# jaekor91/understanding-HMC

Hardware: AMD Instinct MI355X
Metric: leapfrog steps/sec (whole node) + ESS/sec, D=100 MVN at 1M chains (higher is better)
Workload: dtype f64

## Files before the change

understanding-hmc_amd/csrc/hmc_capi.cpp:

```cpp
#include <algorithm>
#include <cmath>
#include <cstdarg>
#include <cstdio>
#include <cstdlib>
#include <mutex>
#include <string>
#include <unordered_map>

#include "hmc.h"
#include "hmc_internal.hpp"
#include "hmc_logit.hpp"
#include "hmc_mix.hpp"

namespace {

thread_local std::string g_err;
#ifdef HMC_DEBUG_HOOKS
unsigned long long* g_stamps = nullptr;
int64_t g_stamp_waves = 0;
#endif

hmc_status fail(hmc_status st, const char* fmt, ...) {
  char buf[512];
  va_list ap;
// ... 163 lines not shown

}

extern "C" {

#ifdef HMC_DEBUG_HOOKS
int64_t hmc_debug_stamps(unsigned long long* host, int64_t cap_words) {
  if (!g_stamps) return 0;
  const int64_t words = g_stamp_waves * hmc::kStampWords < cap_words ? g_stamp_waves * hmc::kStampWords : cap_words;
  if (hipDeviceSynchronize() != hipSuccess) return 0;
  if (hipMemcpy(host, g_stamps, words * sizeof(unsigned long long), hipMemcpyDeviceToHost) != hipSuccess) return 0;
  return words;
}
#endif

const char* hmc_version(void) { return "hmc_amd 0.1.0 gfx950 (diag random kernels, C ABI v1)"; }

const char* hmc_last_error(void) { return g_err.c_str(); }

hmc_status hmc_chain_init(const hmc_target* t, const hmc_kinetic* k, const hmc_schedule* s, const hmc_replay* r,
                          const double* q_start, hmc_state* st, void* stream) {
  if (hmc_status e = check_schedule(t, k, s, false)) return e;
  if (!st) return fail(HMC_EINVAL, "null state");
  if (hmc_status e = check_mass(t, k, s)) return e;
  if (s->n_chains == 0) return HMC_OK;
  if (!st->q || !st->E_prev || !q_start) return fail(HMC_EINVAL, "null state/q_start");
  const bool replay = s->rng_mode == HMC_RNG_REPLAY;
  if (replay && (!r || !r->p0)) return fail(HMC_EINVAL, "replay mode needs p0");
  if (hmc_status e = ws_check(st->order, order_need(t, k, s, st), "hmc_chain_init: state.order")) return e;
  const bool dense = t->kind == HMC_TARGET_DENSE;
  if (hmc::big_path(dense, t->D)) {
    if (!st->order) return fail(HMC_EINVAL, "D=%d needs hmc_random_workspace_size() bytes in state.order", t->D);
    const hmc::Layout lay{0, 0, 0, (t->D + 1) / 2};
    hmc::RandArgs a = rand_args(t, k, s, replay ? r : nullptr, st, lay);
    a.qstart = q_start;
    return hip_status(hmc::launch_big_init(hmc::big_args(a, st->order, dense), dense, replay, (hipStream_t)stream),
                      "hmc_chain_init(large D)");
  }
  if (t->kind == HMC_TARGET_DENSE) {
    const hmc::Layout lay{0, 0, 0, (t->D + 1) / 2};
    hmc::RandArgs a = rand_args(t, k, s, replay ? r : nullptr, st, lay);
    a.qstart = q_start;
    if (st->order) {
      int32_t* valid = reinterpret_cast<int32_t*>(reinterpret_cast<char*>(st->order) +
                                                  hmc::dense_gcache_offset_bytes(s->n_chains) - 16);
      if (hmc_status e = hip_status(hipMemsetAsync(valid, 0, sizeof(int32_t), (hipStream_t)stream), "hmc_chain_init"))
        return e;
    }
    return hip_status(hmc::launch_dense_init(a, replay, (hipStream_t)stream), "hmc_chain_init(dense)");
  }
  const int L_lo = s->L_high > s->L_low ? s->L_low : 5, L_hi = s->L_high > s->L_low ? s->L_high : 20;
  const hmc::Layout lay = hmc::choose_layout(t->D, L_lo, L_hi);
  if (lay.K == 0) return fail(HMC_ENOTSUP, "D=%d too large for the diagonal kernels", t->D);
  hmc::RandArgs a = rand_args(t, k, s, replay ? r : nullptr, st, lay);
  a.qstart = q_start;
  return hip_status(hmc::launch_random_init(a, lay, general_diag(t, k), replay, (hipStream_t)stream),
                    "hmc_chain_init");
}

hmc_status hmc_random_iters(const hmc_target* t, const hmc_kinetic* k, const hmc_schedule* s, const hmc_replay* r,
                            hmc_state* st, void* stream) {
  if (hmc_status e = check_schedule(t, k, s, true)) return e;
  if (!st) return fail(HMC_EINVAL, "null state");
  if (hmc_status e = check_window(t, s, st)) return e;
  if (hmc_status e = check_mass(t, k, s)) return e;
  if (s->iter_begin < 1 || s->iter_end < s->iter_begin || s->iter_end > s->n_iter + 1)
    return fail(HMC_EINVAL, "iteration range must satisfy 1 <= begin <= end <= Niter+1");
  if (s->n_chains == 0) return HMC_OK;
  if (!st->q || !st->E_prev) return fail(HMC_EINVAL, "null state");
  const bool replay = s->rng_mode == HMC_RNG_REPLAY;
  if (replay && (!r || !r->p || !r->L || !r->lnu)) return fail(HMC_EINVAL, "replay mode needs p, L, lnu");
  if (s->n_chains == 0 || s->iter_end == s->iter_begin) return HMC_OK;
  if (st->n_save > 0 && st->traj_q && st->traj_stride < s->L_high)
    return fail(HMC_EINVAL, "traj_stride must be >= L_high");
  if (hmc_status e = ws_check(st->order, order_need(t, k, s, st), "hmc_random_iters: state.order")) return e;
  const bool dense = t->kind == HMC_TARGET_DENSE;
  if (hmc::big_path(dense, t->D)) {
    if (!st->order) return fail(HMC_EINVAL, "D=%d needs hmc_random_workspace_size() bytes in state.order", t->D);
    const hmc::Layout lay{0, 0, 0, (t->D + 1) / 2};
    hmc::RandArgs a = rand_args(t, k, s, replay ? r : nullptr, st, lay);
    return hip_status(hmc::launch_big_iters(hmc::big_args(a, st->order, dense), dense,
                                            s->fp_mode == HMC_MODE_EXACT, replay, (hipStream_t)stream),
                      "hmc_random_iters(large D)");
  }
  if (t->kind == HMC_TARGET_DENSE) {
    const hmc::Layout lay{0, 0, 0, (t->D + 1) / 2};
    hmc::RandArgs a = rand_args(t, k, s, replay ? r : nullptr, st, lay);
    const bool exact = s->fp_mode == HMC_MODE_EXACT;
    int32_t* gvalid = nullptr;
    if (st->order) {
      char* base = reinterpret_cast<char*>(st->order);
      gvalid = reinterpret_cast<int32_t*>(base + hmc::dense_gcache_offset_bytes(s->n_chains) - 16);
      a.gcache = reinterpret_cast<double*>(base + hmc::dense_gcache_offset_bytes(s->n_chains));
      a.gvalid = gvalid;
    }
    auto mark_valid = [&]() -> hmc_status {
      return gvalid ? hip_status(hipMemsetAsync(gvalid, 1, 1, (hipStream_t)stream), "hmc_random_iters") : HMC_OK;
    };
    if (!st->order || a.traj_q || !hmc::dense_order_ok(a)) {
      if (hmc_status e = hip_status(hmc::launch_dense_iters(a, exact, replay, (hipStream_t)stream),
                                    "hmc_random_iters(dense)"))
        return e;
      return mark_valid();
    }
    for (int it = s->iter_begin; it < s->iter_end; ++it) {
      if (hmc_status e = hip_status(hmc::launch_dense_order(a, it, replay, st->order, (hipStream_t)stream),
                                    "hmc_random_iters(dense order)"))
        return e;
      a.it0 = it;
      a.it1 = it + 1;
      a.order = st->order;
      if (hmc_status e = hip_status(hmc::launch_dense_iters(a, exact, replay, (hipStream_t)stream),
                                    "hmc_random_iters(dense)"))
        return e;
      if (hmc_status e = mark_valid()) return e;
    }
    return HMC_OK;
  }
  const hmc::Layout lay = hmc::choose_layout(t->D, s->L_low, s->L_high);
  if (lay.K == 0) return fail(HMC_ENOTSUP, "D=%d too large for the diagonal kernels", t->D);
  hmc::RandArgs a = rand_args(t, k, s, replay ? r : nullptr, st, lay);
  const int64_t lmax = std::max<int64_t>(std::max(s->L_high, 1), a.dbgL > 0 ? a.dbgL : 1);
  const int64_t chunk = std::max<int64_t>(1, 0x7FFFFFFFll / (lmax * lmax));
  for (int it = s->iter_begin; it < s->iter_end;) {
    const int end = (int)std::min<int64_t>(s->iter_end, it + chunk);
    a.it0 = it;
    a.it1 = end;
    if (hmc_status e = hip_status(hmc::launch_random_iters(a, lay, s->fp_mode == HMC_MODE_EXACT, general_diag(t, k),
                                                           replay, (hipStream_t)stream),
                                  "hmc_random_iters"))
      return e;
    it = end;
  }
  return HMC_OK;
}

int32_t hmc_random_leapfrog_form(const hmc_target* t, const hmc_kinetic* k, const hmc_schedule* s) {
  if (!t || !k || !s || t->D < 1 || t->kind == HMC_TARGET_DENSE || hmc::big_path(false, t->D)) return 0;
  const hmc::Layout lay = hmc::choose_layout(t->D, s->L_low, s->L_high);
  if (lay.K == 0) return 0;
  hmc::RandArgs a{};
  a.dt = k->dt;
  return hmc::leapfrog_three_term(a, lay, s->fp_mode == HMC_MODE_EXACT, general_diag(t, k)) ? 1 : 0;
}

hmc_status hmc_random_layout(const hmc_target* t, const hmc_schedule* s, int32_t out[4]) {
  if (!t || !s || !out) return fail(HMC_EINVAL, "hmc_random_layout: null target/schedule/out");
  if (t->D < 1) return fail(HMC_EINVAL, "D must be >= 1");
  if (s->L_high <= s->L_low) return fail(HMC_EINVAL, "L_low must be < L_high (randint)");
  if (t->kind == HMC_TARGET_DENSE) return fail(HMC_ENOTSUP, "hmc_random_layout: dense targets have no such layout");
  if (hmc::big_path(false, t->D)) return fail(HMC_ENOTSUP, "hmc_random_layout: D=%d runs the large-D path", t->D);
  const hmc::Layout lay = hmc::choose_layout(t->D, s->L_low, s->L_high);
  if (lay.K == 0) return fail(HMC_ENOTSUP, "D=%d too large for the diagonal kernels", t->D);
  out[0] = lay.K;
  out[1] = lay.lpc;
  out[2] = lay.cpw;
  out[3] = hmc::wave_layout(lay) ? 1 : 0;
  return HMC_OK;
}

int64_t hmc_random_workspace_size_ex(const hmc_target* t, const hmc_kinetic* k, int64_t n_chains) {
  if (!t || n_chains < 0 || t->D < 1) return 0;
  const bool dense = t->kind == HMC_TARGET_DENSE;
  if (hmc::big_path(dense, t->D)) return hmc::big_workspace_bytes(n_chains, t->D, dense, !k || k->minv_full);
  if (!dense) return 0;
  return hmc::dense_workspace_bytes(n_chains, t->D);
}

int64_t hmc_random_workspace_size(const hmc_target* t, int64_t n_chains) {
  return hmc_random_workspace_size_ex(t, nullptr, n_chains);
}

int64_t hmc_nuts_workspace_size_ex(int32_t D, int64_t n_chains, int32_t d_max, int32_t iters_per_call,
                                   int32_t philox_momenta) {
  if (D < 1 || n_chains < 0 || d_max < 1 || d_max > hmc::kNutsDmaxMax || iters_per_call < 1) return 0;
  int64_t doubles = 0;
  switch (hmc::nuts_kernel(D)) {
    case hmc::NutsKernel::Tree:
      doubles = hmc::nuts_ws_doubles(n_chains, D, d_max, philox_momenta ? iters_per_call : 0);
      break;
    case hmc::NutsKernel::Lock:
      doubles = hmc::nuts_lock_ws_doubles(n_chains, D, d_max, !philox_momenta);
      break;
    case hmc::NutsKernel::PerChain:
      doubles = hmc::nuts_big_ws_doubles(n_chains, D, d_max);
      break;
  }
  return doubles * (int64_t)sizeof(double);
}

int64_t hmc_nuts_workspace_size(int32_t D, int64_t n_chains, int32_t d_max) {
  return std::max(hmc_nuts_workspace_size_ex(D, n_chains, d_max, 32, 1),
                  hmc_nuts_workspace_size_ex(D, n_chains, d_max, 32, 0));
}

static int64_t nuts_need(const hmc_target* t, const hmc_kinetic* k, const hmc_schedule* s) {
  if (s->iter_end <= s->iter_begin || s->n_chains == 0) return 0;
  const int32_t pm = s->rng_mode == HMC_RNG_PHILOX && !k->minv_full ? 1 : 0;
  const int64_t need = hmc_nuts_workspace_size_ex(t->D, s->n_chains, s->d_max, s->iter_end - s->iter_begin, pm);
  return need > 0 ? need : -1;
}

hmc_status hmc_workspace_register(const void* workspace, int64_t bytes) {
  if (!workspace || bytes < 0) return fail(HMC_EINVAL, "hmc_workspace_register: null pointer or negative size");
  ws_record(workspace, bytes);
  return HMC_OK;
}

hmc_status hmc_chain_init_ws(const hmc_target* t, const hmc_kinetic* k, const hmc_schedule* s, const hmc_replay* r,
                             const double* q_start, hmc_state* st, int64_t order_bytes, void* stream) {
  if (hmc_status e = check_schedule(t, k, s, false)) return e;
  if (!st) return fail(HMC_EINVAL, "null state");
  if (!k) return fail(HMC_EINVAL, "null kinetic");
  const int64_t need = order_need(t, k, s, st);
  if (order_bytes < need)
    return fail(HMC_EINVAL, "hmc_chain_init_ws: state.order of %lld bytes, this call needs %lld "
                "(hmc_random_workspace_size_ex)", (long long)order_bytes, (long long)need);
  if (st->order) ws_record(st->order, order_bytes);
  return hmc_chain_init(t, k, s, r, q_start, st, stream);
}

hmc_status hmc_random_iters_ws(const hmc_target* t, const hmc_kinetic* k, const hmc_schedule* s, const hmc_replay* r,
                               hmc_state* st, int64_t order_bytes, void* stream) {
  if (hmc_status e = check_schedule(t, k, s, true)) return e;
  if (!st) return fail(HMC_EINVAL, "null state");
  if (!k) return fail(HMC_EINVAL, "null kinetic");
  const int64_t need = order_need(t, k, s, st);
  if (order_bytes < need)
    return fail(HMC_EINVAL, "hmc_random_iters_ws: state.order of %lld bytes, this call needs %lld "
                "(hmc_random_workspace_size_ex)", (long long)order_bytes, (long long)need);
  if (st->order) ws_record(st->order, order_bytes);
  return hmc_random_iters(t, k, s, r, st, stream);
}

hmc_status hmc_nuts_iters_ws(const hmc_target* t, const hmc_kinetic* k, const hmc_schedule* s, const hmc_replay* r,
                             hmc_state* st, void* workspace, int64_t workspace_bytes, void* stream) {
  if (hmc_status e = check_schedule(t, k, s, false)) return e;
  if (s->d_max < 1 || s->d_max > hmc::kNutsDmaxMax) return fail(HMC_EINVAL, "d_max must be in [1, %d]", hmc::kNutsDmaxMax);
  const int64_t need = nuts_need(t, k, s);
  if (need < 0) return fail(HMC_EINVAL, "NUTS workspace: unsupported D=%d / d_max=%d", t->D, s->d_max);
  if (workspace_bytes < need)
    return fail(HMC_EINVAL, "NUTS workspace of %lld bytes; this call (D=%d, %lld chains, d_max=%d, %d iterations, "
                "%s momenta) needs %lld (hmc_nuts_workspace_size_ex)", (long long)workspace_bytes, t->D,
                (long long)s->n_chains, s->d_max, s->iter_end - s->iter_begin,
                s->rng_mode == HMC_RNG_PHILOX && !k->minv_full ? "Philox" : "no pre-drawn", (long long)need);
  ws_record(workspace, workspace_bytes);
  return hmc_nuts_iters(t, k, s, r, st, workspace, stream);
}

hmc_status hmc_nuts_iters(const hmc_target* t, const hmc_kinetic* k, const hmc_schedule* s, const hmc_replay* r,
                          hmc_state* st, void* workspace, void* stream) {
  if (hmc_status e = check_schedule(t, k, s, false)) return e;
  if (!st) return fail(HMC_EINVAL, "null state");
  if (hmc_status e = check_window(t, s, st)) return e;
  if (s->iter_begin < 1 || s->iter_end < s->iter_begin || s->iter_end > s->n_iter + 1)
    return fail(HMC_EINVAL, "iteration range must satisfy 1 <= begin <= end <= Niter+1");
  if (s->n_chains == 0) return HMC_OK;
  if (!st->q || !st->E_prev) return fail(HMC_EINVAL, "null state");
  if (s->d_max < 1 || s->d_max > hmc::kNutsDmaxMax) return fail(HMC_EINVAL, "d_max must be in [1, %d]", hmc::kNutsDmaxMax);
  if (hmc_status e = check_mass(t, k, s)) return e;
  if (t->kind != HMC_TARGET_DENSE) return fail(HMC_ENOTSUP, "NUTS runs the dense kernel: pass prec as dense");
  const bool replay = s->rng_mode == HMC_RNG_REPLAY;
  if (replay && (!r || !r->p || !r->tape || r->tape_stride < 1)) return fail(HMC_EINVAL, "replay mode needs p and tape");
  if (s->n_chains == 0 || s->iter_end == s->iter_begin) return HMC_OK;
  if (!workspace) return fail(HMC_EINVAL, "null workspace");
  {
    const int64_t need = nuts_need(t, k, s);
    if (need < 0) return fail(HMC_EINVAL, "NUTS workspace: unsupported D=%d / d_max=%d", t->D, s->d_max);
    if (hmc_status e = ws_check(workspace, need, "hmc_nuts_iters: workspace")) return e;
  }
  const hmc::Layout lay{0, 0, 16, (t->D + 1) / 2};
  hmc::RandArgs a = rand_args(t, k, s, replay ? r : nullptr, st, lay);
  a.d_max = s->d_max;
  a.on_dmax = s->on_dmax;
  a.ws = static_cast<double*>(workspace);
  if (replay) {
    a.tape = r->tape;
    a.tape_stride = r->tape_stride;
  }
  a.traj_q = nullptr;
  a.n_save = 0;
  const bool exact = s->fp_mode == HMC_MODE_EXACT;
  switch (hmc::nuts_kernel(t->D)) {
    case hmc::NutsKernel::Lock:
      return hip_status(hmc::launch_nuts_lock(a, exact, replay, (hipStream_t)stream), "hmc_nuts_iters(lockstep)");
    case hmc::NutsKernel::PerChain:
      return hip_status(hmc::launch_nuts_big(a, exact, replay, (hipStream_t)stream), "hmc_nuts_iters(large D)");
    case hmc::NutsKernel::Tree:
      break;
  }
  return hip_status(hmc::launch_nuts_iters(a, exact, replay, (hipStream_t)stream), "hmc_nuts_iters");
}

hmc_status hmc_leapfrog(const hmc_target* t, const hmc_kinetic* k, int64_t n, const double* p, const double* q,
                        double* p_out, double* q_out, int32_t fp_mode, void* stream) {
  if (!t || !k || t->D < 1 || n < 0) return fail(HMC_EINVAL, "bad arguments");
  if (n > 0 && (!p || !q || !p_out || !q_out)) return fail(HMC_EINVAL, "null row pointers");
  if (p_out == p || q_out == q || p_out == q || q_out == p) return fail(HMC_EINVAL, "outputs alias inputs");
  hmc::RowArgs a{};
  a.n = n;
  a.D = t->D;
  a.dense = t->kind == HMC_TARGET_DENSE;
  a.q0 = t->q0;
  a.prec = t->prec;
  if (hmc_status e = check_mass(t, k, nullptr)) return e;
  a.minv = k->minv;
// ... 500 lines not shown
```

understanding-hmc_amd/csrc/hmc_internal.hpp:

```cpp
#pragma once
#include <hip/hip_runtime.h>
#include <stdint.h>

#include "hmc.h"

namespace hmc {

constexpr int kStampWords = 16;

struct Layout {
  int K;
  int lpc;
  int cpw;
  int npairs;
};

struct RandArgs {
  int64_t n;
  int64_t chain_offset;
  int D, npairs, lpc, cpw;
  int niter, wu, thin, Lc, L_low, L_high, it0, it1, i_oob;
  uint32_t k0, k1;
  double dt, h, logc;
  double lf_c, lf_ch, lf_idt2;
  const double* q0;
  const double* prec;
  const double* minv;
  const double* pscale;
  const double* dtv;
  const double* minvf;
  const double* cholt;
  const double* kick;
  const double* rp0;
  const double* rp;
  const double* rlnu;
  const int32_t* rL;
  const double* qstart;
  double* q;
  double* Eprev;
  double* qc;
  double* Ec;
  double* dEc;
  unsigned long long* cnt;
  double* traj_q;
  int32_t* traj_len;
  int32_t* decision;
  int n_save, traj_stride;
  int Lq, q_row0;
  int d_max, on_dmax;
  uint64_t wait_cap;
  int nuts_kb;
  double* ws;
  const double* tape;
  int64_t tape_stride;
  int dbg;
  int dbgL;
  unsigned long long* stamps;
  const int32_t* order;
  double* gcache;
  const int32_t* gvalid;
  int64_t ntiles;
};

using DenseArgs = RandArgs;
int dense_tiles(int D);
constexpr int kNutsDmaxMax = 30;
int64_t nuts_ws_doubles(int64_t n, int D, int d_max, int mom_iters);
hipError_t launch_nuts_iters(const RandArgs& a, bool exact, bool replay, hipStream_t s);
int64_t nuts_big_ws_doubles(int64_t n, int D, int d_max);
bool nuts_lock_path(int D);
int64_t nuts_lock_ws_doubles(int64_t n, int D, int d_max, bool mass);
hipError_t launch_nuts_lock(const RandArgs& a, bool exact, bool replay, hipStream_t s);
hipError_t launch_nuts_big(const RandArgs& a, bool exact, bool replay, hipStream_t s);
enum class NutsKernel { Tree, Lock, PerChain };
inline NutsKernel nuts_kernel(int D) {
  if (dense_tiles(D)) return NutsKernel::Tree;
  return nuts_lock_path(D) ? NutsKernel::Lock : NutsKernel::PerChain;
}

Layout choose_layout(int D, int L_low, int L_high);
bool wave_layout(const Layout& lay);

hipError_t launch_random_init(const RandArgs& a, const Layout& lay, bool gen, bool replay, hipStream_t s);
hipError_t launch_random_iters(const RandArgs& a, const Layout& lay, bool exact, bool gen, bool replay,
                               hipStream_t s);
hipError_t launch_wave_iters(const RandArgs& a, int K, bool exact, bool gen, bool replay, bool three_term,
                             hipStream_t s);
bool leapfrog_three_term(const RandArgs& a, const Layout& lay, bool exact, bool gen);
hipError_t launch_dense_init(const DenseArgs& a, bool replay, hipStream_t s);
hipError_t launch_dense_iters(const DenseArgs& a, bool exact, bool replay, hipStream_t s);
int64_t dense_order_ints(int64_t n);
int64_t dense_gcache_offset_bytes(int64_t n);
int64_t dense_workspace_bytes(int64_t n, int D);
bool dense_order_ok(const DenseArgs& a);
hipError_t launch_dense_order(const DenseArgs& a, int it, bool replay, int32_t* ws, hipStream_t s);
int device_cus();


struct BigArgs {
  RandArgs a;
  double* p;
  double* g;
  double* qi;
  double* gi;
  double* kv;
  double* u;
  const double* gk;
  int32_t* L;
  double* lnu;
  double* E0;
};
bool big_path(int kind_dense, int D);
int64_t big_workspace_bytes(int64_t n, int D, bool dense, bool full_mass);
BigArgs big_args(const RandArgs& a, void* ws, bool dense);
hipError_t launch_big_init(const BigArgs& b, bool dense, bool replay, hipStream_t s);
hipError_t launch_big_iters(const BigArgs& b, bool dense, bool exact, bool replay, hipStream_t s);

struct RowArgs {
  int64_t n;
  int D;
  int dense;
  const double* q0;
  const double* prec;
  const double* minv;
  const double* dtv;
  const double* minvf;
  double dt, logc;
  const double* p;
  const double* q;
  double* po;
  double* qo;
  double* E;
};
hipError_t launch_leapfrog_rows(const RowArgs& a, bool exact, hipStream_t s);
hipError_t launch_energy_rows(const RowArgs& a, hipStream_t s);
hipError_t launch_philox(uint4 c, uint32_t k0, uint32_t k1, int64_t n, uint32_t* out, hipStream_t s);
hipError_t launch_rng_normals(uint32_t k0, uint32_t k1, int64_t chain0, int64_t n, int it, int npairs,
                              double* out, hipStream_t s);

int64_t diag_rowsum_work(int64_t rows, int D);
bool diag_view_ok(int64_t n_chains, int64_t cs, int64_t ss, int n, int D, int halves, int wrap, int slot0);
int64_t diag_variogram_work(int64_t n_chains, int D, int nlags);
int64_t diag_stream_groups(int64_t n_chains);
int64_t diag_conv_work(int64_t n_chains, int D, int T);
hipError_t launch_conv_fused(const double* x, int64_t n_chains, int64_t cs, int64_t ss, int64_t base, int n, int D,
                             int T, double* work, double* out, hipStream_t st);
hipError_t launch_half_sums(const double* x, int64_t n_chains, int64_t cs, int64_t ss, int D, int wrap, int slot0,
                            int n, int T, double* work, double* out, hipStream_t st);
hipError_t launch_stream_accum(const double* x, int64_t n_chains, int64_t cs, int64_t ss, int D, int wrap, int slot0,
                               int carry, int rows, int64_t pos0, int n, double* shift, double* s1, double* s2, int T,
                               double* vpart, double* vsum, hipStream_t st);
hipError_t launch_split_moments(const double* x, int64_t n_chains, int64_t cs, int64_t ss, int64_t base, int n,
                                int D, double* mean_out, double* std_out, hipStream_t st);
hipError_t launch_rowsum(const double* x, int64_t n_outer, int64_t os, int64_t n_inner, int64_t is, int64_t base,
                         int D, const double* center, double* work, double* out, hipStream_t st);
hipError_t launch_variogram(const double* x, int64_t n_chains, int64_t cs, int64_t ss, int64_t base, int n, int D,
                            int t0, int t1, double* work, double* out, hipStream_t st);

}
```

understanding-hmc_amd/csrc/hmc_random.hip:

```cpp
#include <cstdlib>

#include "hmc_device.hpp"
#include "hmc_internal.hpp"
#include "hmc_target_ops.hpp"

namespace hmc {

namespace {

__device__ __forceinline__ unsigned long long stamp(bool on) {
  return on ? __builtin_amdgcn_s_memtime() : 0ull;
}

struct Lane {
  int lane, g, s, base;
  int64_t c;
  bool active;
  bool leader;
};

__device__ __forceinline__ Lane lane_info(const RandArgs& a) {
  Lane L;
  L.lane = threadIdx.x & (kWave - 1);
  const int64_t wave = (int64_t)blockIdx.x * (blockDim.x / kWave) + (threadIdx.x / kWave);
// ... 247 lines not shown
      ph[5] += t_6 - t_5;
    }
  }

#pragma unroll
  for (int j = 0; j < K; ++j)
    if (pv[j]) store_pair(a.q + ln.c * (int64_t)a.D, kk[j], even, 2 * kk[j] + 1 < a.D, q[2 * j], q[2 * j + 1]);
  if (ln.leader) a.Eprev[ln.c] = Eprev;
  if (a.stamps && ln.lane == 0) {
    const int64_t wv = (int64_t)blockIdx.x * (blockDim.x / kWave) + (threadIdx.x / kWave);
#pragma unroll
    for (int i = 0; i < 6; ++i) a.stamps[wv * kStampWords + i] = ph[i];
    a.stamps[wv * kStampWords + 6] = t_start;
    a.stamps[wv * kStampWords + 7] = stamp(true);
    const unsigned hwid = __builtin_amdgcn_s_getreg((31 << 11) | 4);
    const unsigned xcc = __builtin_amdgcn_s_getreg((31 << 11) | 20);
    a.stamps[wv * kStampWords + 5] = ((unsigned long long)hwid << 32) | ((unsigned long long)(xcc & 0xffff) << 16) |
                           (a.stamps[wv * kStampWords + 5] & 0xffffull);
  }
  n_acc = wave_sum_u64(n_acc);
  n_acc_wu = wave_sum_u64(n_acc_wu);
  n_lf = wave_sum_u64(n_lf);
  n_lf2 = wave_sum_u64(n_lf2);
  n_oob = wave_sum_u64(n_oob);
  if (ln.lane == 0 && a.cnt) {
    const int64_t wv = (int64_t)blockIdx.x * (blockDim.x / kWave) + (threadIdx.x / kWave);
    unsigned long long* cs = a.cnt + (wv & (HMC_COUNTER_SLOTS - 1)) * HMC_NCOUNTERS;
    if (n_acc) atomicAdd(cs + HMC_CNT_ACCEPT, n_acc);
    if (n_acc_wu) atomicAdd(cs + HMC_CNT_ACCEPT_WU, n_acc_wu);
    if (n_lf) atomicAdd(cs + HMC_CNT_LEAPFROG, n_lf);
    if (n_lf2) atomicAdd(cs + HMC_CNT_LEAPFROG_SQ, n_lf2);
    if (n_oob) atomicAdd(cs + HMC_CNT_OOB_REJECT, n_oob);
  }
}

template <int K>
hipError_t launch_init_k(const RandArgs& a, bool gen, bool replay, dim3 grid, hipStream_t s) {
  if (gen) {
    if (replay) k_random_init<K, true, true><<<grid, 256, 0, s>>>(a);
    else k_random_init<K, true, false><<<grid, 256, 0, s>>>(a);
  } else {
    if (replay) k_random_init<K, false, true><<<grid, 256, 0, s>>>(a);
    else k_random_init<K, false, false><<<grid, 256, 0, s>>>(a);
  }
  return hipGetLastError();
}

template <int K, bool EXACT>
hipError_t launch_iters_k2(const RandArgs& a, bool gen, bool replay, dim3 grid, hipStream_t s) {
  if (gen) {
    if (replay) k_random_iters<K, EXACT, true, true><<<grid, 256, 0, s>>>(a);
    else k_random_iters<K, EXACT, true, false><<<grid, 256, 0, s>>>(a);
  } else {
    if (replay) k_random_iters<K, EXACT, false, true><<<grid, 256, 0, s>>>(a);
    else k_random_iters<K, EXACT, false, false><<<grid, 256, 0, s>>>(a);
  }
  return hipGetLastError();
}

template <int K>
hipError_t launch_iters_k(const RandArgs& a, bool exact, bool gen, bool replay, dim3 grid, hipStream_t s) {
  return exact ? launch_iters_k2<K, true>(a, gen, replay, grid, s)
               : launch_iters_k2<K, false>(a, gen, replay, grid, s);
}

dim3 grid_for(const RandArgs& a) {
  const int64_t waves = (a.n + a.cpw - 1) / a.cpw;
  return dim3((unsigned)((waves + 3) / 4));
}

}

static double expected_max(int lo, int hi, int c) {
  const int n = hi - lo;
  if (n <= 1 || c <= 1) return 0.5 * (lo + hi - 1);
  double e = 0.0, prev = 0.0;
  for (int x = lo; x < hi; ++x) {
    const double F = pow((double)(x - lo + 1) / n, c);
    e += x * (F - prev);
    prev = F;
  }
  return e;
}

Layout choose_layout(int D, int L_low, int L_high) {
  static const int Ks[] = {1, 2, 4, 5, 8, 16};
  Layout best{0, 0, 0, (D + 1) / 2};
#ifdef HMC_DEBUG_HOOKS
  if (const char* fk = getenv("HMC_FORCE_K")) {
    const int K = atoi(fk);
    const int lpc = (best.npairs + K - 1) / K;
    for (int k : Ks)
      if (k == K && lpc <= kWave) return Layout{K, lpc, kWave / lpc, best.npairs};
  }
#endif
  if (best.npairs > kWave / 2) {
    for (int K : {1, 2, 4, 8, 16})
      if (K * kWave >= best.npairs) return Layout{K, kWave, 1, best.npairs};
    return best;
  }
  double best_score = -1.0;
  const double mean = 0.5 * (L_low + L_high - 1);
  for (int K : Ks) {
    const int lpc = (best.npairs + K - 1) / K;
    if (lpc > kWave) continue;
    const int cpw = kWave / lpc;
    const double util = (double)best.npairs * cpw / (kWave * (double)K);
    const double emax = expected_max(L_low, L_high, cpw);
    const double score = util * (emax > 0 ? mean / emax : 1.0);
    if (score > best_score + 1e-9) {
      best_score = score;
      best.K = K;
      best.lpc = lpc;
      best.cpw = cpw;
    }
  }
  return best;
}

hipError_t launch_random_init(const RandArgs& a, const Layout& lay, bool gen, bool replay, hipStream_t s) {
  const dim3 grid = grid_for(a);
  switch (lay.K) {
    case 1: return launch_init_k<1>(a, gen, replay, grid, s);
    case 2: return launch_init_k<2>(a, gen, replay, grid, s);
    case 4: return launch_init_k<4>(a, gen, replay, grid, s);
    case 5: return launch_init_k<5>(a, gen, replay, grid, s);
    case 8: return launch_init_k<8>(a, gen, replay, grid, s);
    case 16: return launch_init_k<16>(a, gen, replay, grid, s);
  }
  return hipErrorInvalidValue;
}

bool wave_layout(const Layout& lay) {
#ifdef HMC_DEBUG_HOOKS
  const char* kern = getenv("HMC_KERNEL");
  const bool force_group = kern && kern[0] == 'g';
#else
  const bool force_group = false;
#endif
  return lay.cpw == 1 && !force_group && (lay.K == 1 || lay.K == 2 || lay.K == 4 || lay.K == 8 || lay.K == 16);
}

bool leapfrog_three_term(const RandArgs& a, const Layout& lay, bool exact, bool gen) {
#ifdef HMC_NO_THREE_TERM
  return false;
#else
  constexpr double kThreeTermMinDtw = 1e-3;
  if (exact || gen || !wave_layout(lay)) return false;
  const double dtw2 = a.dt * a.dt;
  return dtw2 >= kThreeTermMinDtw * kThreeTermMinDtw && dtw2 < 4.0;
#endif
}

hipError_t launch_random_iters(const RandArgs& a, const Layout& lay, bool exact, bool gen, bool replay,
                               hipStream_t s) {
  if (wave_layout(lay))
    return launch_wave_iters(a, lay.K, exact, gen, replay, leapfrog_three_term(a, lay, exact, gen), s);
  const dim3 grid = grid_for(a);
  switch (lay.K) {
    case 1: return launch_iters_k<1>(a, exact, gen, replay, grid, s);
    case 2: return launch_iters_k<2>(a, exact, gen, replay, grid, s);
    case 4: return launch_iters_k<4>(a, exact, gen, replay, grid, s);
    case 5: return launch_iters_k<5>(a, exact, gen, replay, grid, s);
    case 8: return launch_iters_k<8>(a, exact, gen, replay, grid, s);
    case 16: return launch_iters_k<16>(a, exact, gen, replay, grid, s);
  }
  return hipErrorInvalidValue;
}

}
```

Baseline: 35.00 billion.

## Add 16-lane-per-chain rows kernel for D≈100 diagonal random-L HMC

Adds a specialised kernel for D in 97..112 that places four chains per wave, each spread across 16 lanes holding seven coordinates per lane. Momentum is generated through a per-chain LDS ring buffer, and leapfrog runs as a hand-written three-term FMA loop in inline asm that masks out lanes with shorter trajectories. Energy sums use DPP row reductions, accept and reject is done with ballots, and energy rows are buffered for nontemporal stores. The goal is better lane utilisation and less per-step overhead than the generic wave layout for D=100, in exchange for a lot of fragile, shape-specific assembly.

Result: faster. 38.66 billion (median of 6 runs) (+10.5%).

```diff
diff --git a/understanding-hmc_amd/csrc/hmc_capi.cpp b/understanding-hmc_amd/csrc/hmc_capi.cpp
--- a/understanding-hmc_amd/csrc/hmc_capi.cpp
+++ b/understanding-hmc_amd/csrc/hmc_capi.cpp
@@ -339,6 +339,14 @@
   if (hmc::big_path(false, t->D)) return fail(HMC_ENOTSUP, "hmc_random_layout: D=%d runs the large-D path", t->D);
   const hmc::Layout lay = hmc::choose_layout(t->D, s->L_low, s->L_high);
   if (lay.K == 0) return fail(HMC_ENOTSUP, "D=%d too large for the diagonal kernels", t->D);
+  if (hmc::rows_shape(t->D, s->L_low, s->L_high) && s->fp_mode != HMC_MODE_EXACT && s->rng_mode != HMC_RNG_REPLAY &&
+      !t->q0 && !t->prec) {
+    out[0] = 4;
+    out[1] = 16;
+    out[2] = 4;
+    out[3] = 0;
+    return HMC_OK;
+  }
   out[0] = lay.K;
   out[1] = lay.lpc;
   out[2] = lay.cpw;
diff --git a/understanding-hmc_amd/csrc/hmc_internal.hpp b/understanding-hmc_amd/csrc/hmc_internal.hpp
--- a/understanding-hmc_amd/csrc/hmc_internal.hpp
+++ b/understanding-hmc_amd/csrc/hmc_internal.hpp
@@ -87,6 +87,9 @@
 hipError_t launch_wave_iters(const RandArgs& a, int K, bool exact, bool gen, bool replay, bool three_term,
                              hipStream_t s);
 bool leapfrog_three_term(const RandArgs& a, const Layout& lay, bool exact, bool gen);
+bool rows_shape(int D, int L_low, int L_high);
+bool rows_kernel(const RandArgs& a, const Layout& lay, bool exact, bool gen, bool replay);
+hipError_t launch_rows_iters(const RandArgs& a, hipStream_t s);
 hipError_t launch_dense_init(const DenseArgs& a, bool replay, hipStream_t s);
 hipError_t launch_dense_iters(const DenseArgs& a, bool exact, bool replay, hipStream_t s);
 int64_t dense_order_ints(int64_t n);
diff --git a/understanding-hmc_amd/csrc/hmc_random.hip b/understanding-hmc_amd/csrc/hmc_random.hip
--- a/understanding-hmc_amd/csrc/hmc_random.hip
+++ b/understanding-hmc_amd/csrc/hmc_random.hip
@@ -423,8 +423,23 @@
 #endif
 }
 
+bool rows_shape(int D, int L_low, int L_high) {
+#ifdef HMC_NO_ROWS
+  return false;
+#else
+  return D >= 97 && D <= 112 && L_low >= 1 && L_high <= (1 << 12);
+#endif
+}
+
+bool rows_kernel(const RandArgs& a, const Layout& lay, bool exact, bool gen, bool replay) {
+  const bool full = a.traj_q != nullptr || a.dbg != 0 || a.dbgL >= 0;
+  if (replay || full || !rows_shape(a.D, a.L_low, a.L_high) || !leapfrog_three_term(a, lay, exact, gen)) return false;
+  return !a.qc || 4 * (int64_t)a.Lq * a.D * 8 < (int64_t)1 << 31;
+}
+
 hipError_t launch_random_iters(const RandArgs& a, const Layout& lay, bool exact, bool gen, bool replay,
                                hipStream_t s) {
+  if (rows_kernel(a, lay, exact, gen, replay)) return launch_rows_iters(a, s);
   if (wave_layout(lay))
     return launch_wave_iters(a, lay.K, exact, gen, replay, leapfrog_three_term(a, lay, exact, gen), s);
   const dim3 grid = grid_for(a);
diff --git a/understanding-hmc_amd/csrc/hmc_rows.hip b/understanding-hmc_amd/csrc/hmc_rows.hip
--- /dev/null
+++ b/understanding-hmc_amd/csrc/hmc_rows.hip
@@ -0,0 +1,326 @@
+#include "hmc_device.hpp"
+#include "hmc_internal.hpp"
+#include "hmc_target_ops.hpp"
+
+namespace hmc {
+
+namespace {
+
+constexpr int kRowLanes = 16;
+constexpr int kRowChains = kWave / kRowLanes;
+constexpr int kRowsBlock = 512;
+constexpr int kRowChunkBytes = 8 * kRowLanes;
+constexpr uint32_t kRowRingBytes = 10 * kRowChunkBytes;
+constexpr uint32_t kRowRingAlloc = 11 * kRowChunkBytes;
+constexpr size_t kRowsLds =
+    8 * (size_t)kNormalTableDoubles + (size_t)(kRowsBlock / kWave) * kRowChains * kRowRingAlloc;
+
+template <int C>
+__device__ __forceinline__ double rows_sumsq(const double (&v)[C], double s0) {
+  double s = __builtin_fma(v[1], v[1], s0);
+  s = __builtin_fma(v[0], v[0], s);
+#pragma unroll
+  for (int e = 2; e < C; ++e) s = __builtin_fma(v[e], v[e], s);
+  return s;
+}
+
+__device__ __forceinline__ double row_sum_l15(double v) {
+  v += dpp_u<0x111>(v);
+  v += dpp_u<0x112>(v);
+  v += dpp_u<0x114>(v);
+  v += dpp_u<0x118>(v);
+  return v;
+}
+
+__device__ __forceinline__ int s_max_i32(int a, int b) {
+  int r;
+  asm("s_max_i32 %0, %1, %2" : "=s"(r) : "s"(a), "s"(b) : "scc");
+  return r;
+}
+
+__device__ __forceinline__ void add_mask(uint32_t& n, uint64_t mask) {
+  uint64_t co;
+  asm("v_addc_co_u32_e64 %0, %1, %0, 0, %2" : "+v"(n), "=&s"(co) : "s"(mask));
+}
+
+__device__ __forceinline__ double park_row_shift(double buf, double v) {
+  const int lo = __builtin_amdgcn_update_dpp(__double2loint(v), __double2loint(buf), 0x101, 0xF, 0xF, false);
+  const int hi = __builtin_amdgcn_update_dpp(__double2hiint(v), __double2hiint(buf), 0x101, 0xF, 0xF, false);
+  return __hiloint2double(hi, lo);
+}
+
+template <int C>
+__global__ __launch_bounds__(kRowsBlock) __attribute__((amdgpu_waves_per_eu(4, 4))) void k_rows_iters(RandArgs a) {
+  static_assert(C == 7, "seven coordinates per lane: D in (96, 112], only the last slot is partial");
+  extern __shared__ __attribute__((aligned(16))) double s_rows[];
+  double* const s_ntab = s_rows;
+  char* const ring_b = reinterpret_cast<char*>(s_rows + kNormalTableDoubles);
+  init_normal_tables(s_ntab);
+  __syncthreads();
+  const int lane = threadIdx.x & (kWave - 1);
+  const int wib = threadIdx.x / kWave;
+  const int64_t c0 = (int64_t)kRowChains * uniform_i(blockIdx.x * (kRowsBlock / kWave) + wib);
+  if (c0 >= a.n) return;
+  const int r = lane / kRowLanes, s = lane & (kRowLanes - 1);
+  const int64_t c = c0 + r;
+  const bool valid = c < a.n;
+  const bool v6 = s + kRowLanes * (C - 1) < a.D;
+  const bool st6 = valid && v6;
+  const uint64_t gc = (uint64_t)(a.chain_offset + c);
+  const uint32_t ringrow = (uint32_t)(wib * kRowChains + r) * kRowRingAlloc;
+
+  int gen_n = 0;
+  uint32_t gposb = 0;
+  uint32_t gk = s, git = a.it0;
+  const uint32_t wlane = ringrow + 16 * s;
+  int rbaseb = 0;
+  const int dpb = 16 * a.npairs;
+  const uint32_t rlane = ringrow + 8 * s;
+  double q[C], p[C], qi[C];
+  auto advance = [&](uint32_t& k, uint32_t& i) {
+    uint64_t bo;
+    uint32_t tk;
+    asm("v_add_u32_e32 %0, 16, %0\n\t"
+        "v_subrev_co_u32_e32 %2, vcc, %4, %0\n\t"
+        "v_subb_co_u32_e64 %1, %3, %1, -1, vcc\n\t"
+        "v_cndmask_b32_e32 %0, %2, %0, vcc"
+        : "+v"(k), "+v"(i), "=&v"(tk), "=&s"(bo)
+        : "s"(a.npairs)
+        : "vcc");
+  };
+  auto ring_momentum = [&](int it) {
+    const int need = (it - a.it0 + 1) * a.npairs;
+    while (gen_n < need) {
+      double z0, z1;
+      normal_pair_tab(draw_block(gk, git, gc, a.k0, a.k1), s_ntab, z0, z1);
+      char* const w = ring_b + (gposb + wlane);
+      *reinterpret_cast<double2*>(w) = make_double2(z0, z1);
+      if (gposb == 0 && s < kRowLanes / 2) *reinterpret_cast<double2*>(w + kRowRingBytes) = make_double2(z0, z1);
+      gen_n += kRowLanes;
+      gposb += 16 * kRowLanes;
+      if (gposb >= kRowRingBytes) gposb -= kRowRingBytes;
+      advance(gk, git);
+    }
+    __builtin_amdgcn_wave_barrier();
+    const uint32_t cbb = (uint32_t)rbaseb & ~(uint32_t)(kRowChunkBytes - 1);
+    const uint32_t a0 = ((uint32_t)rbaseb - cbb) + rlane;
+#pragma unroll
+    for (int j = 0; j < C; ++j) {
+      uint32_t cj = cbb + kRowChunkBytes * j;
+      if (cj >= kRowRingBytes) cj -= kRowRingBytes;
+      p[j] = *reinterpret_cast<const double*>(ring_b + (opaque_s32(cj) + a0));
+    }
+    p[C - 1] = v6 ? p[C - 1] : 0.0;
+    rbaseb += dpb;
+    if (rbaseb >= (int)kRowRingBytes) rbaseb -= kRowRingBytes;
+  };
+
+  double* const qst = a.q + c * (int64_t)a.D + s;
+#pragma unroll
+  for (int j = 0; j < C; ++j) {
+    q[j] = 0.0;
+    if (j < C - 1 ? valid : st6) q[j] = qst[kRowLanes * j];
+  }
+  double Eprev = valid ? a.Eprev[c] : 0.0;
+  __builtin_amdgcn_s_waitcnt(0x0F70);
+
+  ring_momentum(a.it0);
+  const double hlogc = 0.5 * a.logc;
+  double m0l = rows_sumsq<C>(q, 0.0);
+  double e0l = rows_sumsq<C>(p, m0l);
+  double E0 = 0.0;
+
+  int row = 0, phase = 0;
+  if (a.it0 >= a.wu) {
+    row = (a.it0 - a.wu) / a.thin;
+    phase = (a.it0 - a.wu) - row * a.thin;
+  }
+  int qslot = row % a.Lq;
+  double Ebuf = 0.0, dEbuf = 0.0;
+  int row_first = 0, nbuf = 0;
+  const uint32_t bprow = (uint32_t)(lane & ~(kRowLanes - 1)) * 4;
+  double* const Ec = a.Ec ? a.Ec + c * (int64_t)a.Lc + s : nullptr;
+  double* const dEc = a.dEc ? a.dEc + c * (int64_t)a.Lc + s : nullptr;
+  char* const qcb = a.qc ? reinterpret_cast<char*>(a.qc + c0 * (int64_t)a.Lq * a.D) : nullptr;
+  const uint32_t qoff = (uint32_t)(r * a.Lq * a.D + s) * 8u;
+  auto flush_E = [&](int n) {
+    const int first = kRowLanes - n;
+    if (valid && s >= first) {
+      if (Ec) __builtin_nontemporal_store(Ebuf, Ec + (row_first - first));
+      if (dEc) __builtin_nontemporal_store(dEbuf, dEc + (row_first - first));
+    }
+  };
+  uint32_t n_acc = 0, n_acc_wu = 0, n_lf = 0, n_lf2 = 0, n_oob = 0;
+  int it_base = a.it0 - kRowLanes, draw_L = 0;
+  double draw_lnu = 0.0;
+
+  int L_nxt = 0;
+  double lnu_nxt = 0.0;
+  auto fetch_L = [&](int it) {
+    if (it - it_base >= kRowLanes) {
+      it_base = it;
+      const uint4 rr = draw_block(kDrawSlot, (uint32_t)(it + s), gc, a.k0, a.k1);
+      draw_L = uniform_int(rr.x, a.L_low, a.L_high);
+      const double u = u53(rr.z, rr.w);
+      draw_lnu = u > 0.0 ? fast_log(u) : -__builtin_inf();
+      draw_lnu *= 2.0;
+    }
+    const int bsrc = (int)(bprow + 4u * (uint32_t)(it - it_base));
+    L_nxt = __builtin_amdgcn_ds_bpermute(bsrc, draw_L);
+    lnu_nxt = __hiloint2double(__builtin_amdgcn_ds_bpermute(bsrc, __double2hiint(draw_lnu)),
+                               __builtin_amdgcn_ds_bpermute(bsrc, __double2loint(draw_lnu)));
+  };
+
+  auto iteration = [&](auto post_c, int it) {
+    constexpr bool post = decltype(post_c)::value;
+    const bool write_row = post && ((it == a.niter) || (phase == a.thin - 1));
+    fetch_L(it);
+    const int L = L_nxt;
+    const double lnu = lnu_nxt;
+#pragma unroll
+    for (int e = 0; e < C; ++e) asm("v_mov_b64 %0, %1" : "=v"(qi[e]) : "v"(q[e]));
+    double (&x)[C] = p;
+    const uint32_t oddm = (uint32_t)__builtin_amdgcn_sbfe(L, 0, 1);
+    const uint32_t dtlo = __double2loint(a.dt), dthi = __double2hiint(a.dt);
+    const double sh = __hiloint2double(__double2hiint(a.h) ^ ((uint32_t)L << 31), __double2loint(a.h));
+    const double sq = __hiloint2double(dthi & oddm, dtlo & oddm);
+    const double sx = a.dt - sq;
+#pragma unroll
+    for (int e = 0; e < C; ++e) {
+      double t;
+      asm("v_fma_f64 %0, %1, %2, %3" : "=v"(t) : "v"(sh), "v"(q[e]), "v"(p[e]));
+      x[e] = __builtin_fma(-sx, t, q[e]);
+      q[e] = __builtin_fma(sq, t, q[e]);
+    }
+    const int np = L >> 1;
+    const int np_max = s_max_i32(s_max_i32(__builtin_amdgcn_readlane(np, 0), __builtin_amdgcn_readlane(np, 16)),
+                                 s_max_i32(__builtin_amdgcn_readlane(np, 32), __builtin_amdgcn_readlane(np, 48)));
+    if (np_max > 0) {
+      int i;
+      asm volatile("s_mov_b32 %[i], 0\n"
+                   "1:\n\t"
+                   "v_cmpx_lt_i32_e32 vcc, %[i], %[np]\n\t"
+                   "v_fma_f64 %[x0], %[c], %[q0], -%[x0]\n\t"
+                   "v_fma_f64 %[x1], %[c], %[q1], -%[x1]\n\t"
+                   "v_fma_f64 %[x2], %[c], %[q2], -%[x2]\n\t"
+                   "v_fma_f64 %[x3], %[c], %[q3], -%[x3]\n\t"
+                   "v_fma_f64 %[x4], %[c], %[q4], -%[x4]\n\t"
+                   "v_fma_f64 %[x5], %[c], %[q5], -%[x5]\n\t"
+                   "v_fma_f64 %[x6], %[c], %[q6], -%[x6]\n\t"
+                   "v_fma_f64 %[q0], %[c], %[x0], -%[q0]\n\t"
+                   "v_fma_f64 %[q1], %[c], %[x1], -%[q1]\n\t"
+                   "v_fma_f64 %[q2], %[c], %[x2], -%[q2]\n\t"
+                   "v_fma_f64 %[q3], %[c], %[x3], -%[q3]\n\t"
+                   "v_fma_f64 %[q4], %[c], %[x4], -%[q4]\n\t"
+                   "v_fma_f64 %[q5], %[c], %[x5], -%[q5]\n\t"
+                   "v_fma_f64 %[q6], %[c], %[x6], -%[q6]\n\t"
+                   "s_add_i32 %[i], %[i], 1\n\t"
+                   "s_cmp_lt_i32 %[i], %[n]\n\t"
+                   "s_cbranch_scc1 1b\n\t"
+                   "s_mov_b64 exec, -1"
+                   : [x0] "+v"(x[0]), [x1] "+v"(x[1]), [x2] "+v"(x[2]), [x3] "+v"(x[3]), [x4] "+v"(x[4]),
+                     [x5] "+v"(x[5]), [x6] "+v"(x[6]), [q0] "+v"(q[0]), [q1] "+v"(q[1]), [q2] "+v"(q[2]),
+                     [q3] "+v"(q[3]), [q4] "+v"(q[4]), [q5] "+v"(q[5]), [q6] "+v"(q[6]), [i] "=&s"(i)
+                   : [np] "v"(np), [c] "s"(a.lf_c), [n] "s"(np_max)
+                   : "vcc", "scc");
+    }
+    double w[C];
+#pragma unroll
+    for (int e = 0; e < C; ++e) w[e] = __builtin_fma(a.lf_ch, q[e], -x[e]);
+    double m1l = rows_sumsq<C>(q, 0.0);
+    const double k1 = __builtin_fma(rows_sumsq<C>(w, 0.0), a.lf_idt2, m1l);
+    const double s2 = row_sum_l15(k1 - e0l);
+    const double se = row_sum_l15(e0l);
+    E0 = __builtin_fma(se, 0.5, hlogc);
+    if (write_row) {
+      if (nbuf == 0) row_first = row;
+      Ebuf = park_row_shift(Ebuf, E0);
+      dEbuf = park_row_shift(dEbuf, E0 - Eprev);
+      if (++nbuf == kRowLanes) {
+        flush_E(kRowLanes);
+        nbuf = 0;
+      }
+    }
+    Eprev = E0;
+    if (it + 1 < a.it1) ring_momentum(it + 1);
+    const uint64_t b15 = (__builtin_amdgcn_ballot_w64(s2 < 0.0) | __builtin_amdgcn_ballot_w64(lnu < -s2)) &
+                         0x8000800080008000ull;
+    const uint64_t accm = (b15 << 1) - (b15 >> 15);
+    const uint64_t rej = ~accm;
+    if (rej != 0) {
+      uint64_t ex;
+      asm volatile("s_mov_b64 %[ex], exec\n\t"
+                   "s_mov_b64 exec, %[rej]\n\t"
+                   "v_mov_b64 %[q0], %[i0]\n\t"
+                   "v_mov_b64 %[q1], %[i1]\n\t"
+                   "v_mov_b64 %[q2], %[i2]\n\t"
+                   "v_mov_b64 %[q3], %[i3]\n\t"
+                   "v_mov_b64 %[q4], %[i4]\n\t"
+                   "v_mov_b64 %[q5], %[i5]\n\t"
+                   "v_mov_b64 %[q6], %[i6]\n\t"
+                   "v_mov_b64 %[m1], %[m0]\n\t"
+                   "s_mov_b64 exec, %[ex]"
+                   : [q0] "+v"(q[0]), [q1] "+v"(q[1]), [q2] "+v"(q[2]), [q3] "+v"(q[3]), [q4] "+v"(q[4]),
+                     [q5] "+v"(q[5]), [q6] "+v"(q[6]), [m1] "+v"(m1l), [ex] "=&s"(ex)
+                   : [rej] "s"(rej), [i0] "v"(qi[0]), [i1] "v"(qi[1]), [i2] "v"(qi[2]), [i3] "v"(qi[3]),
+                     [i4] "v"(qi[4]), [i5] "v"(qi[5]), [i6] "v"(qi[6]), [m0] "v"(m0l));
+    }
+    m0l = m1l;
+    if (write_row && qcb && row >= a.q_row0) {
+      char* const rowb = qcb + (int64_t)qslot * a.D * 8;
+#pragma unroll
+      for (int j = 0; j < C; ++j)
+        if (j < C - 1 ? valid : st6)
+          __builtin_nontemporal_store(q[j], reinterpret_cast<double*>(rowb + qoff) + kRowLanes * j);
+    }
+    if (post) add_mask(n_acc, accm); else add_mask(n_acc_wu, accm);
+    add_mask(n_oob, it < a.i_oob ? rej : 0ull);
+    n_lf += (uint32_t)L;
+    n_lf2 += __umul24((uint32_t)L, (uint32_t)L);
+    e0l = rows_sumsq<C>(p, m0l);
+    if (post && ++phase == a.thin) {
+      phase = 0;
+      ++row;
+      if (++qslot == a.Lq) qslot = 0;
+    }
+  };
+  const int it_mid = min(max(a.wu, a.it0), a.it1);
+  for (int it = a.it0; it < it_mid; ++it) iteration(std::false_type{}, it);
+  for (int it = it_mid; it < a.it1; ++it) iteration(std::true_type{}, it);
+
+  if (nbuf > 0) flush_E(nbuf);
+#pragma unroll
+  for (int j = 0; j < C; ++j)
+    if (j < C - 1 ? valid : st6) qst[kRowLanes * j] = q[j];
+  if (valid && s == kRowLanes - 1) {
+    a.Eprev[c] = Eprev;
+    if (a.cnt) {
+      unsigned long long* cs = a.cnt + (c & (HMC_COUNTER_SLOTS - 1)) * HMC_NCOUNTERS;
+      if (n_acc) atomicAdd(cs + HMC_CNT_ACCEPT, (unsigned long long)n_acc);
+      if (n_acc_wu) atomicAdd(cs + HMC_CNT_ACCEPT_WU, (unsigned long long)n_acc_wu);
+      if (n_lf) atomicAdd(cs + HMC_CNT_LEAPFROG, (unsigned long long)n_lf);
+      if (n_lf2) atomicAdd(cs + HMC_CNT_LEAPFROG_SQ, (unsigned long long)n_lf2);
+      if (n_oob) atomicAdd(cs + HMC_CNT_OOB_REJECT, (unsigned long long)n_oob);
+    }
+  }
+}
+
+}
+
+hipError_t launch_rows_iters(const RandArgs& a, hipStream_t s) {
+  static bool raised[64] = {};
+  int dev = 0;
+  if (hipError_t e = hipGetDevice(&dev)) return e;
+  if (dev < 0 || dev >= 64 || !raised[dev]) {
+    if (hipError_t e = hipFuncSetAttribute(reinterpret_cast<const void*>(&k_rows_iters<7>),
+                                           hipFuncAttributeMaxDynamicSharedMemorySize, (int)kRowsLds))
+      return e;
+    if (dev >= 0 && dev < 64) raised[dev] = true;
+  }
+  constexpr int chains_per_block = (kRowsBlock / kWave) * kRowChains;
+  const dim3 grid((unsigned)((a.n + chains_per_block - 1) / chains_per_block));
+  k_rows_iters<7><<<grid, kRowsBlock, kRowsLds, s>>>(a);
+  return hipGetLastError();
+}
+
+}
```
